# FangjinhuaWang/PatchmatchNet

Hardware: AMD Instinct MI355X
Metric: depth-maps/sec at 1600x1200 N=5 src views (higher is better)
Workload: dtype f32

## Files before the change

include/pmn_hip.h:

```cpp
#ifndef PMN_HIP_H
#define PMN_HIP_H

#include <stdint.h>

#ifdef __cplusplus
extern "C" {
#endif

#define PMN_ABI_VERSION 25
#define PMN_MLP_FLOATS 340
#define PMN_MAX_DEPTH 64
#define PMN_MAX_NEIGHBORS 17
#define PMN_MAX_FUSE_SRC 32
#define PMN_TSDF_MAX_VIEWS 16
#define PMN_TSDF_MARK_SPAN 8
#define PMN_RASTER_MAX_DIM 16384
#define PMN_RASTER_MAX_BOX 64
#define PMN_SPLAT_MAX_RADIUS 32

#define PMN_OK 0
#define PMN_ERR_ARG (-1)
#define PMN_ERR_SHAPE (-2)
#define PMN_ERR_LAUNCH (-3)

int pmn_abi_version(void);

const char *pmn_error_string(int code);

int pmn_nchw_to_nhwc(const float *in, float *out, int B, int C, int h, int w, void *stream);

int pmn_feature_weight(const float *ref_nhwc, const float *eval_offsets, const int *eval_table_host,
                       const float *mlp, int B, int C, int G, int K, int h, int w,
                       float *out_feature_weight, void *stream);

int pmn_init_hypotheses(const float *noise, const float *depth, int depth_shift, const float *depth_min,
                        const float *depth_max, int num_sample, float interval_scale, const float *propa_offsets,
                        const int *propa_table_host, int K, int B, int h, int w, float *depth_sample,
                        float *xnorm, void *stream);

int pmn_warp_correlate(const float *ref_nhwc, const float *src_nhwc, const float *rel_proj,
                       const float *depth_sample, const float *view_weights_in, int vw_shift,
                       const float *similarity_mlp, const float *pixelwise_mlp, int B, int N, int C,
                       int G, int D, int h, int w, int hs, int ws, float *cost_out, float *view_weights_out,
                       int *vw_argmax_out, float *similarity_out, void *stream);

int pmn_warp_correlate_views(const float *ref_nhwc, const void *src_view_table, const float *rel_proj,
                             const float *depth_sample, const float *view_weights_in, int vw_shift,
                             const float *similarity_mlp, const float *pixelwise_mlp, int B, int N, int C,
                             int G, int D, int h, int w, int hs, int ws, float *cost_out, float *view_weights_out,
                             int *vw_argmax_out, float *similarity_out, void *stream);

int pmn_aggregate_regress(const float *cost, const float *depth_sample, const float *xnorm,
                          const float *feature_weight, const float *eval_offsets, const int *eval_table_host,
                          int K, float interval_scale, int is_inverse, int B, int D, int h, int w,
                          float *score_out, float *depth_out, void *stream);

int pmn_confidence(const float *score, int B, int D, int h, int w, int H, int W, float *confidence_out,
                   int *depth_index_out, void *stream);

int pmn_conv2d(const float *in, const float *weights, const float *shift, const float *up, float *out, int N, int H,
               int W, int cin, int cout, int K, int stride, int pad, int dil, int relu, int in_nchw, int out_nchw,
               int up_h, int up_w, void *stream);

int pmn_fpn_tail(const float *x, const float *up, const float *w_in, const float *b_in, const float *w_out, float *out,
                 int N, int H, int W, int cin, int cmid, int cout, void *stream);

int pmn_conv2d_mfma(const float *in, const float *weights, const float *shift, float *out, float *out_b, int N, int H, int W,
                    int cin, int cout, int ca, int K, int stride, int pad, int dil, int relu, int planar, void *stream);


int pmn_conv2d_f16s(const float *in, const void *weights, const float *shift, float *out, int N, int H, int W, int cin, int cout,
                    int k, int stride, int relu, void *stream);

int pmn_conv2d_f16s_pair(const float *in, const void *weights_a, const float *shift_a, const void *weights_b, const float *shift_b,
                         float *out, int N, int H, int W, int channels, int relu, void *stream);

int pmn_offset_heads_f16s(const float *in, const void *weights, const float *shift, float *out_a, float *out_b, int N, int H, int W,
                          int cin, int cout, int ca, int dil, void *stream);

int pmn_fpn_level(const float *x, const float *u, const float *w, const float *b, float *out_a, float *out_b, int N, int H,
                  int W, int cin, int cout, int ca, void *stream);

int pmn_deconv3x3s2(const float *in, const float *weights, const float *shift, float *out, int N, int Hi, int Wi, int cin,
                    int cout, int relu, void *stream);

int pmn_refine_front(const float *img, const float *t2, const float *w0, const float *s0, const float *wd, const float *sd,
                     float *x16, int B, int H, int W, void *stream);
int pmn_refine_tail(const float *x16, const float *w3, const float *s3, const float *wr, const float *dnorm,
                    const float *depth_min, const float *depth_max, float *out, int B, int H, int W, void *stream);

int pmn_refine_fused(const float *img, const float *t2, const float *w0, const float *s0, const float *wd, const float *sd,
                     const void *w3a, const float *s3, const float *wr, const float *dnorm, const float *depth_min,
                     const float *depth_max, float *out, int B, int H, int W, void *stream);

int pmn_stage_projections(const float *intrinsics, const float *extrinsics, int B, int V, int nstages, float scale0,
                          float *rel, void *stream);

int pmn_stem(const float *img, const float *w0, const float *s0, const float *w1, const float *s1, float *out, int N, int H,
             int W, void *stream);

int pmn_stem_f16s(const float *img, const float *w0, const float *s0, const void *w1a, const float *s1, float *out, int N, int H,
                  int W, void *stream);

int pmn_stem_f16s_views(const float *const *img_table, int views, const float *w0, const float *s0, const void *w1a,
                        const float *s1, float *out, int B, int H, int W, void *stream);

int pmn_stem_conv2_f16s(const float *img, const float *w0, const float *s0, const void *w1a, const float *s1, const void *w2b,
                        const float *s2, float *out, int N, int H, int W, void *stream);

int pmn_stem_conv2_f16s_views(const float *const *img_table, int views, const float *w0, const float *s0, const void *w1a,
                              const float *s1, const void *w2b, const float *s2, float *out, int B, int H, int W, void *stream);

int pmn_differentiable_warping(const float *src_nchw, const float *rel_proj, const float *depth, int B, int C,
                               int D, int h, int w, int hs, int ws, float *warped, void *stream);

int pmn_fuse_view(const float *maps, long long slot_stride, int ref_slot, const int *src_slots_host,
                  const int *src_hw_host, int n_src, const float *mats, int H, int W, float geo_pixel_thres, float geo_depth_thres, int geo_mask_thres,
                  float photo_thres, unsigned char *masks, float *xyz, double *depth_avg, int *geo_sum, void *stream);

int pmn_fuse_view_merged(const float *maps, long long slot_stride, int ref_slot, const int *src_slots_host,
                         const int *src_hw_host, int n_src, const float *mats, int H, int W, float geo_pixel_thres,
// ... 197 lines not shown
```

patchmatchnet_amd/_lib.py:

```python
from __future__ import annotations

import ctypes
import os
import subprocess
from typing import Optional

_CSRC = os.path.join(os.path.dirname(os.path.abspath(__file__)), "csrc")
LIB_PATH = os.path.join(_CSRC, "libpmn_hip.so")
ABI_VERSION = 25
MLP_FLOATS = 340
MAX_DEPTH = 64
MAX_NEIGHBORS = 17
MAX_FUSE_SRC = 32
TSDF_MAX_VIEWS = 16
TSDF_MARK_SPAN = 8
RASTER_MAX_DIM = 16384
RASTER_MAX_BOX = 64
SPLAT_MAX_RADIUS = 32
ICP_SUMS = 17
ICP_LIMBS = 5
ICP_BLOCK_POINTS = 256
VOXEL_LONG_RUN = 256
VOXEL_MAX_CHANNELS = 8
CROP_MAX_VERTICES = 4096
MESH_PLACE_LONG_RUN = 256
MESH_SIMPLIFY_MAX_FACES = 715827882
MESH_SMOOTH_LONG_ROW = 256
MESH_SMOOTH_MAX_STEPS = 65536
NORMAL_SWEEPS = 6
NORMAL_MAX_VIEWPOINTS = 4096
PLANE_MAX_HYPOTHESES = 4096
PLANE_SUMS = 10
PLANE_LIMBS = 5
PLANE_BLOCK_POINTS = 1024
MLS_QUADRIC_MIN = 6
MLS_PIVOT_MIN = 1e-10

_fp = ctypes.c_void_p
_ip = ctypes.c_void_p
_hp = ctypes.c_void_p
_i = ctypes.c_int
_f = ctypes.c_float
_s = ctypes.c_void_p

SIGNATURES = {
    "pmn_abi_version": [],
    "pmn_error_string": [_i],
    "pmn_nchw_to_nhwc": [_fp, _fp, _i, _i, _i, _i, _s],
    "pmn_feature_weight": [_fp, _fp, _hp, _fp, _i, _i, _i, _i, _i, _i, _fp, _s],
    "pmn_init_hypotheses": [_fp, _fp, _i, _fp, _fp, _i, _f, _fp, _hp, _i, _i, _i, _i, _fp, _fp, _s],
    "pmn_warp_correlate": [_fp, _fp, _fp, _fp, _fp, _i, _fp, _fp, _i, _i, _i, _i, _i, _i, _i, _i, _i, _fp, _fp, _ip,
                           _fp, _s],
    "pmn_warp_correlate_views": [_fp, _fp, _fp, _fp, _fp, _i, _fp, _fp, _i, _i, _i, _i, _i, _i, _i, _i, _i, _fp, _fp, _ip,
                                 _fp, _s],
    "pmn_aggregate_regress": [_fp, _fp, _fp, _fp, _fp, _hp, _i, _f, _i, _i, _i, _i, _i, _fp, _fp, _s],
    "pmn_confidence": [_fp, _i, _i, _i, _i, _i, _i, _fp, _ip, _s],
    "pmn_conv2d": [_fp, _fp, _fp, _fp, _fp] + [_i] * 14 + [_s],
    "pmn_fpn_tail": [_fp] * 6 + [_i] * 6 + [_s],
    "pmn_fpn_level": [_fp] * 6 + [_i] * 6 + [_s],
    "pmn_conv2d_f16s": [_fp] * 4 + [_i] * 8 + [_s],
    "pmn_offset_heads_f16s": [_fp] * 5 + [_i] * 7 + [_s],
    "pmn_conv2d_f16s_pair": [_fp] * 6 + [_i] * 5 + [_s],
    "pmn_refine_front": [_fp] * 7 + [_i] * 3 + [_s],
    "pmn_refine_tail": [_fp] * 8 + [_i] * 3 + [_s],
    "pmn_refine_fused": [_fp] * 13 + [_i] * 3 + [_s],
    "pmn_conv2d_mfma": [_fp] * 5 + [_i] * 12 + [_s],
    "pmn_deconv3x3s2": [_fp] * 4 + [_i] * 6 + [_s],
    "pmn_stage_projections": [_fp, _fp, _i, _i, _i, _f, _fp, _s],
    "pmn_stem": [_fp] * 6 + [_i] * 3 + [_s],
    "pmn_stem_f16s": [_fp] * 6 + [_i] * 3 + [_s],
    "pmn_stem_f16s_views": [_fp, _i] + [_fp] * 5 + [_i] * 3 + [_s],
    "pmn_stem_conv2_f16s": [_fp] * 8 + [_i] * 3 + [_s],
    "pmn_stem_conv2_f16s_views": [_fp, _i] + [_fp] * 7 + [_i] * 3 + [_s],
    "pmn_differentiable_warping": [_fp, _fp, _fp, _i, _i, _i, _i, _i, _i, _i, _fp, _s],
    "pmn_fuse_view": [_fp, ctypes.c_longlong, _i, _hp, _hp, _i, _fp, _i, _i, _f, _f, _i, _f, _fp, _fp, _fp, _ip, _s],
    "pmn_fuse_view_merged": [_fp, ctypes.c_longlong, _i, _hp, _hp, _i, _fp, _i, _i, _f, _f, _i, _f, _fp, _fp, _fp, _ip, _fp,
                             ctypes.c_longlong, _fp, _s],
    "pmn_pack_points": [_fp, _fp, _fp, _i, _i, _i, _fp, ctypes.c_longlong, _fp, _ip, _fp, _s],
    "pmn_pack_points_normals": [_fp, _fp, _fp, _fp, _i, _fp, _i, _i, _i, _fp, ctypes.c_longlong, _fp, _ip, _fp, _s],
    "pmn_depth_normals": [_fp, _i, _i, _hp, _i, _f, _fp, _s],
    "pmn_normalize_depth": [_fp, _fp, _fp, _i, _i, _fp, _s],
    "pmn_check_f16_domain": [_fp, ctypes.c_longlong, _ip, _s],
    "pmn_plan_create": [ctypes.POINTER(ctypes.c_void_p)],
    "pmn_plan_begin": [_hp],
    "pmn_plan_end": [_hp],
    "pmn_plan_count": [_hp],
    "pmn_plan_kernel_name": [_hp, _i],
    "pmn_plan_launch": [_hp, _s],
    "pmn_plan_destroy": [_hp],
    "pmn_plan_fork": [_hp],
    "pmn_plan_switch": [_hp, _i],
    "pmn_plan_join": [_hp],
    "pmn_plan_entry_branch": [_hp, _i],
    "pmn_plan_launch_part": [_hp, _i, _s],
    "pmn_view_scores": [_fp] * 6 + [_i, _i, ctypes.c_longlong, ctypes.c_longlong] + [ctypes.c_double] * 3 + [_fp, _s],
    "pmn_depth_metrics": [_fp, _fp, _hp, _hp, _hp, _i, _hp, _i, _i, _i, _i, _fp, ctypes.c_longlong, _fp, _s],
    "pmn_nn_distance": [_fp, _ip, ctypes.c_longlong, _hp, ctypes.c_double, _hp, _fp, _ip, ctypes.c_longlong, ctypes.c_double, _fp, _ip,
                        _s],
    "pmn_reduce_round": [_fp, _ip, ctypes.c_longlong, _hp, ctypes.c_double, _hp, ctypes.c_double, _ip, _ip, _ip, _s],
    "pmn_tsdf_integrate": [_fp] * 4 + [_hp, _hp, _f, _f, _fp, ctypes.c_longlong] + [_hp] * 5 + [_i, _s],
    "pmn_mt_count": [_fp, _fp, _hp, _f, _ip, _ip, _s],
    "pmn_mt_emit": [_fp] * 4 + [_hp, _hp, _f, _f] + [_ip] * 4 + [_fp, _ip, _fp, _ip, _s],
    "pmn_tsdf_mark_blocks": [_ip, _ip, _hp, _hp, _f, _f, _fp, ctypes.c_longlong] + [_hp] * 4 + [_i, _s],
    "pmn_tsdf_integrate_blocks": [_fp] * 4 + [_ip, _i, _hp, _hp, _f, _f, _fp, ctypes.c_longlong] + [_hp] * 5 + [_i, _s],
    "pmn_mt_count_blocks": [_fp, _fp, _ip, _ip, _i, _hp, _f, _ip, _ip, _s],
    "pmn_mt_emit_blocks": [_fp] * 4 + [_ip, _ip, _i, _hp, _hp, _f, _f] + [_ip] * 4 + [_fp, _ip, _fp, _ip, _s],
    "pmn_raster_triangles": [_fp, _i, _ip, _i, _hp, _i, _i, ctypes.c_longlong, _ip, _ip, _ip, _s],
    "pmn_splat_points": [_fp, ctypes.c_longlong, _hp, _i, _i, _f, _f, _ip, _ip, _s],
    "pmn_raster_resolve": [_ip, _i, _i, _hp, _fp, ctypes.c_longlong, _ip, ctypes.c_longlong, _ip, _fp, _i, _fp, _ip, _ip, _fp, _s],
    "pmn_icp_accumulate": [_fp, _ip, ctypes.c_longlong, _hp, ctypes.c_double, _hp, _fp, _ip, ctypes.c_longlong, _hp, _hp, ctypes.c_double,
                           _fp, ctypes.c_longlong, _fp, _s],
    "pmn_voxel_mean": [_fp, _fp, _i, ctypes.c_longlong, _ip, ctypes.c_longlong, _fp, _fp, _s],
    "pmn_crop_prism": [_fp, ctypes.c_longlong, _fp, _i, _i, ctypes.c_double, ctypes.c_double, _hp, _ip, _s],
    "pmn_mesh_components": [_ip, _i, _i, _ip, _ip, _s],
    "pmn_mesh_face_samples": [_fp, _i, _ip, _i, ctypes.c_double, ctypes.c_ulonglong, _ip, _ip, _s],
    "pmn_mesh_sample": [_fp, _i, _ip, _i, _ip, _ip, ctypes.c_longlong, ctypes.c_ulonglong, _fp, _ip, _ip, _s],
    "pmn_undistort_image": [_fp, _i, _i, _i, _i, _hp, _hp, _i, _i, _fp, _fp, _fp, _s],
    "pmn_knn_distance": [_fp, _ip, ctypes.c_longlong, _hp, ctypes.c_double, _hp, _fp, _ip, ctypes.c_longlong, _i, ctypes.c_double, _i,
                         _fp, _ip, _fp, _s],
    "pmn_radius_count": [_fp, _ip, ctypes.c_longlong, _hp, ctypes.c_double, _hp, _fp, _ip, ctypes.c_longlong, ctypes.c_double, _i, _ip,
                         _s],
    "pmn_knn_normals": [_fp, _ip, ctypes.c_longlong, _hp, ctypes.c_double, _hp, _fp, _ip, ctypes.c_longlong, _i, ctypes.c_double, _i,
                        _fp, _i, ctypes.c_double, _fp, _fp, _ip, _s],
    "pmn_cloud_core": [_fp, _ip, ctypes.c_longlong, _hp, ctypes.c_double, _hp, ctypes.c_double, ctypes.c_longlong, _ip, _s],
    "pmn_cloud_dbscan": [_fp, _ip, ctypes.c_longlong, _hp, ctypes.c_double, _hp, ctypes.c_double, _ip, _ip, _ip, _ip, _s],
    "pmn_plane_score": [_fp, _fp, _ip, ctypes.c_longlong, _fp, _i, ctypes.c_double, ctypes.c_double, _ip, _s],
    "pmn_plane_inliers": [_fp, _fp, _ip, ctypes.c_longlong, _hp, ctypes.c_double, ctypes.c_double, _hp, _hp, _fp, ctypes.c_longlong, _ip,
                          _fp, _s],
    "pmn_cloud_sdf_blocks": [_fp, _ip, ctypes.c_longlong, _hp, ctypes.c_double, _hp, _fp, _ip, _ip, _i, _hp, _hp, _f, _f, _i,
                             ctypes.c_double, ctypes.c_double, _fp, _fp, _fp, _fp, _s],
    "pmn_knn_mls": [_fp, _ip, ctypes.c_longlong, _hp, ctypes.c_double, _hp, _fp, _ip, ctypes.c_longlong, _i, ctypes.c_double, _i, _i,
                    ctypes.c_double, _fp, _fp, _fp, _ip, _ip, _s],
    "pmn_mesh_distance": [_fp, _ip, ctypes.c_longlong, _hp, ctypes.c_double, _hp, _ip, ctypes.c_double, _fp, _i, _ip, _i, _fp, _ip,
# ... 80 lines not shown
```

patchmatchnet_amd/csrc/hypotheses.hip:

```cpp
#include <cstring>

#include "pmn_common.hpp"
#define PMN_DIV48(u) ((u) / 48.0f)
#define PMN_DIV48R(u) pmn_div_by((u), 48.0f, r48)

struct HypArgs {
    const float* noise;
    const float* depth;
    const float* depth_min;
    const float* depth_max;
    const float* offsets;
    float* depth_sample;
    float* xnorm;
    int depth_shift, num_sample, K, B, h, w;
    float interval_scale;
    int table[2 * PMN_MAX_NEIGHBORS];
};

__device__ __forceinline__ float centre_hypothesis(const HypArgs& a, int b, int qy, int qx, float inv_min, float inv_max,
                                                   float interval, int kc) {
#pragma clang fp contract(off)
    const int h = a.h, w = a.w;
    if (a.noise) {
        const float u = a.noise[((size_t)b * 48 + 24) * h * w + (size_t)qy * w + qx] + 24.0f;
// ... 155 lines not shown
                v[j] = pmn_div(1.0f, inv);
            }
        }
    }

    if constexpr (KT > 0) {
        constexpr int KB = KT < 8 ? KT : 8;
        static_assert(KT % KB == 0, "whole batches");
        const float* cbase = from_noise ? a.noise + ((size_t)b * 48 + 24) * hw
                                        : a.depth + (size_t)b * (h >> a.depth_shift) * ws;
        const int sh = from_noise ? 0 : a.depth_shift, cw = from_noise ? w : ws;
#pragma unroll
        for (int k0b = 0; k0b < KT; k0b += KB) {
            float ox[KB], oy[KB];
#pragma unroll
            for (int i = 0; i < KB; ++i) {
                ox[i] = a.offsets[((size_t)b * 2 * KT + 2 * (k0b + i)) * hw + p];
                oy[i] = a.offsets[((size_t)b * 2 * KT + 2 * (k0b + i) + 1) * hw + p];
            }
            PmnTaps t[KB];
            float c[KB][4];
#pragma unroll
            for (int i = 0; i < KB; ++i) {
                float ix, iy;
                pmn_neighbor_position((float)x, (float)y, a.table[2 * (k0b + i)], a.table[2 * (k0b + i) + 1], ox[i], oy[i], h, w, ix,
                                      iy);
                t[i] = pmn_make_taps(ix, iy, h, w);
                const int qy = t[i].off / w, qx = t[i].off - qy * w;
                c[i][0] = cbase[(size_t)(qy >> sh) * cw + (qx >> sh)];
                c[i][1] = cbase[(size_t)(qy >> sh) * cw + ((qx + 1) >> sh)];
                c[i][2] = cbase[(size_t)((qy + 1) >> sh) * cw + (qx >> sh)];
                c[i][3] = cbase[(size_t)((qy + 1) >> sh) * cw + ((qx + 1) >> sh)];
            }
#pragma unroll
            for (int i = 0; i < KB; ++i) {
                float cc[4];
#pragma unroll
                for (int q = 0; q < 4; ++q) {
                    if (from_noise) {
                        const float inv = inv_max + PMN_DIV48R(c[i][q] + 24.0f) * (inv_min - inv_max);
                        cc[q] = pmn_div(1.0f, inv);
                    } else if (a.num_sample == 1) {
                        cc[q] = c[i][q];
                    } else {
                        float inv = pmn_div(1.0f, c[i][q]) + interval * (float)kc;
                        inv = fminf(fmaxf(inv, inv_max), inv_min);
                        cc[q] = pmn_div(1.0f, inv);
                    }
                }
                v[D0T + k0b + i] = fmaf(cc[3], t[i].w11, fmaf(cc[2], t[i].w10, fmaf(cc[1], t[i].w01, cc[0] * t[i].w00)));
            }
        }
#pragma unroll
        for (int kk = 2; kk <= NP2; kk <<= 1) {
#pragma unroll
            for (int jj = kk >> 1; jj > 0; jj >>= 1) {
#pragma unroll
                for (int i = 0; i < NP2; ++i) {
                    const int l = i ^ jj;
                    if (l > i) {
                        const float lo = fminf(v[i], v[l]), hi = fmaxf(v[i], v[l]);
                        if ((i & kk) == 0) {
                            v[i] = lo;
                            v[l] = hi;
                        } else {
                            v[i] = hi;
                            v[l] = lo;
                        }
                    }
                }
            }
        }
    }

    const float range = inv_min - inv_max, rrange = pmn_rcp_refined(range);
#pragma unroll
    for (int j = 0; j < D; ++j) {
        const size_t o = ((size_t)b * D + j) * hw + p;
        a.depth_sample[o] = v[j];
        a.xnorm[((size_t)b * hw + p) * D + j] = pmn_div_by(pmn_div(1.0f, v[j]) - inv_max, range, rrange);
    }
}

extern "C" int pmn_init_hypotheses(const float* noise, const float* depth, int depth_shift, const float* depth_min,
                                   const float* depth_max, int num_sample, float interval_scale,
                                   const float* propa_offsets, const int* propa_table_host, int K, int B, int h, int w,
                                   float* depth_sample, float* xnorm, void* stream) {
    if ((!noise && !depth) || !depth_min || !depth_max || !depth_sample || !xnorm) return PMN_ERR_ARG;
    if (B < 1 || h < 2 || w < 2 || K < 0 || depth_shift < 0 || depth_shift > 1) return PMN_ERR_ARG;
    if (K > 0 && (!propa_offsets || !propa_table_host)) return PMN_ERR_ARG;
    if (K > 16) return PMN_ERR_SHAPE;
    if (!noise && num_sample < 1) return PMN_ERR_ARG;
    if (depth_shift && ((h | w) & 1)) return PMN_ERR_ARG;
    const int D0 = noise ? 48 : num_sample;
    const int D = D0 + K;
    if (D > PMN_MAX_DEPTH) return PMN_ERR_SHAPE;
    HypArgs a;
    memset(&a, 0, sizeof(a));
    a.noise = noise;
    a.depth = noise ? nullptr : depth;
    a.depth_min = depth_min;
    a.depth_max = depth_max;
    a.offsets = propa_offsets;
    a.depth_sample = depth_sample;
    a.xnorm = xnorm;
    a.depth_shift = depth_shift;
    a.num_sample = noise ? 48 : num_sample;
    a.K = K;
    a.B = B; a.h = h; a.w = w;
    a.interval_scale = interval_scale;
    for (int i = 0; i < 2 * K; ++i) a.table[i] = propa_table_host[i];
    const int bs = (h * w <= 64 * 1024) ? 64 : PMN_BLOCK;
    const dim3 grid((h * w + bs - 1) / bs, B), block(bs);
    hipStream_t s = (hipStream_t)stream;
    if (noise && K == 16) PMN_LAUNCH((init_hypotheses_fixed_kernel<64, 48, 16>), grid, block, 0, s, a);
    else if (!noise && num_sample == 16 && K == 16) PMN_LAUNCH((init_hypotheses_fixed_kernel<32, 16, 16>), grid, block, 0, s, a);
    else if (!noise && num_sample == 8 && K == 8) PMN_LAUNCH((init_hypotheses_fixed_kernel<16, 8, 8>), grid, block, 0, s, a);
    else if (!noise && num_sample == 8 && K == 0) PMN_LAUNCH((init_hypotheses_fixed_kernel<8, 8, 0>), grid, block, 0, s, a);
    else if (D <= 8) PMN_LAUNCH(init_hypotheses_kernel<8>, grid, block, 0, s, a);
    else if (D <= 16) PMN_LAUNCH(init_hypotheses_kernel<16>, grid, block, 0, s, a);
    else if (D <= 32) PMN_LAUNCH(init_hypotheses_kernel<32>, grid, block, 0, s, a);
    else PMN_LAUNCH(init_hypotheses_kernel<64>, grid, block, 0, s, a);
    PMN_CHECK_LAUNCH();
    return PMN_OK;
}
```

patchmatchnet_amd/ops.py:

```python
from __future__ import annotations

import ctypes
import threading
from typing import List, Optional, Sequence, Tuple

import numpy as np
import torch

from . import _lib
from ._lib import PmnError, check


_TIMING = None
_TIMING_ON = True


def enable_kernel_timing() -> None:
    global _TIMING, _TIMING_ON
    _TIMING, _TIMING_ON = [], True


def pause_kernel_timing(paused: bool) -> None:
    global _TIMING_ON
    _TIMING_ON = not paused
# ... 197 lines not shown
        if v.is_contiguous():
            return v
        x = x.contiguous()
    _dev(x, "x")
    B, C, h, w = x.shape
    if out is None:
        out = torch.empty((B, h, w, C), dtype=torch.float32, device=x.device)
    else:
        _dev(out, "out")
        if tuple(out.shape) != (B, h, w, C):
            raise PmnError("nchw_to_nhwc: bad output shape")
    _note((x,), (out,))
    with torch.cuda.device(x.device):
        check(_lib.lib().pmn_nchw_to_nhwc(x.data_ptr(), out.data_ptr(), B, C, h, w, _stream(x)), "pmn_nchw_to_nhwc")
    return out


def stack_sources_nhwc(src_features: Sequence[torch.Tensor]) -> torch.Tensor:
    buf, sizes = stack_sources_padded(src_features)
    if any(sz != sizes[0] for sz in sizes):
        raise PmnError("all source feature maps of one stage must share a shape (stack_sources_padded handles mixed sizes)")
    return buf


def stack_sources_padded(src_features: Sequence[torch.Tensor]):
    if len(src_features) == 0:
        raise PmnError("at least one source view is required")
    B, C = src_features[0].shape[:2]
    sizes = [(int(f.shape[2]), int(f.shape[3])) for f in src_features]
    if any(tuple(f.shape[:2]) != (B, C) for f in src_features):
        raise PmnError("source feature maps of one stage must share batch size and channels")
    hs, ws = max(h for h, _ in sizes), max(w for _, w in sizes)
    mixed = any(sz != (hs, ws) for sz in sizes)
    alloc = torch.zeros if mixed else torch.empty
    buf = alloc((len(src_features), B, hs, ws, C), dtype=torch.float32, device=src_features[0].device)
    for i, f in enumerate(src_features):
        v = f.permute(0, 2, 3, 1)
        if sizes[i] != (hs, ws):
            _dev(f.contiguous(), "src_feature")
            buf[i][:, :sizes[i][0], :sizes[i][1], :].copy_(v)
        elif f.is_cuda and f.dtype == torch.float32 and v.is_contiguous():
            buf[i].copy_(v)
        else:
            nchw_to_nhwc(f.contiguous(), buf[i])
    return buf, sizes


def rescale_projection_rows(rel_proj: torch.Tensor, sizes, padded_hw) -> torch.Tensor:
    HS, WS = padded_hw
    if all(sz == (HS, WS) for sz in sizes):
        return rel_proj
    out = rel_proj.clone()
    for v, (h_v, w_v) in enumerate(sizes):
        if (h_v, w_v) != (HS, WS):
            out[:, v, 0, :] *= (w_v - 1) / (WS - 1)
            out[:, v, 1, :] *= (h_v - 1) / (HS - 1)
    return out.contiguous()


def _mlp_dev(t: torch.Tensor, name: str) -> torch.Tensor:
    _dev(t, name)
    if t.numel() != _lib.MLP_FLOATS:
        raise PmnError(f"{name}: expected a packed MLP block of {_lib.MLP_FLOATS} floats")
    return t


def feature_weight(ref_nhwc: torch.Tensor, eval_offsets: torch.Tensor, table: np.ndarray, mlp: torch.Tensor,
                   G: int) -> torch.Tensor:
    _dev(ref_nhwc, "ref_nhwc")
    _dev(eval_offsets, "eval_offsets")
    B, h, w, C = ref_nhwc.shape
    K = eval_offsets.shape[1] // 2
    if tuple(eval_offsets.shape) != (B, 2 * K, h, w):
        raise PmnError("feature_weight: eval_offsets must be [B,2K,h,w]")
    tab, tab_p = _host_i32(table, 2 * K, "table")
    _mlp_dev(mlp, "mlp")
    out = torch.empty((B, K, h, w), dtype=torch.float32, device=ref_nhwc.device)
    _note((ref_nhwc, eval_offsets, mlp), (out,))
    with torch.cuda.device(ref_nhwc.device):
        check(_lib.lib().pmn_feature_weight(ref_nhwc.data_ptr(), eval_offsets.data_ptr(), tab_p, mlp.data_ptr(), B, C, G,
                                            K, h, w,
                                            out.data_ptr(), _stream(out)), "pmn_feature_weight")
    return out


def init_hypotheses(noise: Optional[torch.Tensor], depth: Optional[torch.Tensor], depth_shift: int,
                    depth_min: torch.Tensor, depth_max: torch.Tensor, num_sample: int, interval_scale: float,
                    propa_offsets: Optional[torch.Tensor], table: Optional[np.ndarray], h: int, w: int
                    ) -> Tuple[torch.Tensor, torch.Tensor]:
    _dev(depth_min, "depth_min")
    _dev(depth_max, "depth_max")
    B = depth_min.shape[0]
    dev = depth_min.device
    if noise is not None:
        _dev(noise, "noise")
        if tuple(noise.shape) != (B, 48, h, w):
            raise PmnError("init_hypotheses: noise must be [B,48,h,w]")
        D0 = 48
    else:
        if depth is None:
            raise PmnError("init_hypotheses: need noise or depth")
        _dev(depth, "depth")
        if tuple(depth.shape) != (B, 1, h >> depth_shift, w >> depth_shift):
            raise PmnError(f"init_hypotheses: depth must be [B,1,{h >> depth_shift},{w >> depth_shift}], "
                           f"got {tuple(depth.shape)}")
        D0 = num_sample
    K = 0
    tab_p = None
    tab = None
    if propa_offsets is not None:
        _dev(propa_offsets, "propa_offsets")
        K = propa_offsets.shape[1] // 2
        if tuple(propa_offsets.shape) != (B, 2 * K, h, w):
            raise PmnError("init_hypotheses: propa_offsets must be [B,2K,h,w]")
        tab, tab_p = _host_i32(table, 2 * K, "table")
    D = D0 + K
    ds = torch.empty((B, D, h, w), dtype=torch.float32, device=dev)
    xn = torch.empty((B, h, w, D), dtype=torch.float32, device=dev).permute(0, 3, 1, 2)
    _note((noise, depth if noise is None else None, depth_min, depth_max, propa_offsets), (ds, xn))
    with torch.cuda.device(dev):
        check(_lib.lib().pmn_init_hypotheses(_ptr(noise), _ptr(depth) if noise is None else None, depth_shift,
                                             depth_min.data_ptr(), depth_max.data_ptr(), num_sample,
                                             float(interval_scale), _ptr(propa_offsets), tab_p, K, B, h, w,
                                             ds.data_ptr(), xn.data_ptr(), _stream(ds)), "pmn_init_hypotheses")
    del tab
    return ds, xn


class SourceTable:

    def __init__(self, table: torch.Tensor, shape) -> None:
        if table.dtype != torch.int64 or not table.is_cuda or table.numel() != int(shape[0]):
            raise PmnError("SourceTable: int64 device tensor with one address per source view")
        self.table, self.shape, self.device = table, tuple(int(x) for x in shape), table.device

    @staticmethod
    def image_in_place(im: torch.Tensor) -> bool:
        return bool(im.is_cuda and im.dtype == torch.float32 and im.is_contiguous() and im.data_ptr() % 16 == 0)

    @staticmethod
    def addresses(maps) -> list:
        out = []
        for m in maps:
            if not (m.is_cuda and m.dtype == torch.float32 and m.is_contiguous()):
                raise PmnError("SourceTable: dense float32 channels-last device maps")
            out.append(m.data_ptr())
        return out


def warp_correlate(ref_nhwc: torch.Tensor, src_nhwc, rel_proj: torch.Tensor, depth_sample: torch.Tensor,
                   view_weights: Optional[torch.Tensor], vw_shift: int, similarity_mlp: torch.Tensor,
                   pixelwise_mlp: Optional[torch.Tensor], G: int, want_similarity: bool = False,
                   want_argmax: bool = False):
    _dev(ref_nhwc, "ref_nhwc")
    table = src_nhwc if isinstance(src_nhwc, SourceTable) else None
    if table is None:
        _dev(src_nhwc, "src_nhwc")
    _dev(rel_proj, "rel_proj")
    _dev(depth_sample, "depth_sample")
    B, h, w, C = ref_nhwc.shape
    N, Bs, hs, ws, Cs = src_nhwc.shape
    D = depth_sample.shape[1]
    if Bs != B or Cs != C or tuple(depth_sample.shape) != (B, D, h, w) or tuple(rel_proj.shape) != (B, N, 4, 4):
        raise PmnError("warp_correlate: inconsistent shapes")
    dev = ref_nhwc.device
    sim_p = _mlp_dev(similarity_mlp, "similarity_mlp").data_ptr()
    pix_p, vw_out, argmax = None, None, None
    if view_weights is not None:
        _dev(view_weights, "view_weights")
        if tuple(view_weights.shape) != (B, N, h >> vw_shift, w >> vw_shift):
            raise PmnError("Patchmatch Evaluation: Different number of images and view weights")
    else:
        if pixelwise_mlp is None:
            raise PmnError("warp_correlate: pixelwise_mlp required when view_weights is None")
        pix_p = _mlp_dev(pixelwise_mlp, "pixelwise_mlp").data_ptr()
        vw_out = torch.empty((B, N, h, w), dtype=torch.float32, device=dev)
        if want_argmax:
            argmax = torch.empty((B, N, h, w), dtype=torch.int32, device=dev)
    cost = torch.empty((B, h, w, D), dtype=torch.float32, device=dev).permute(0, 3, 1, 2)
    sim = torch.empty((B, G, D, h, w), dtype=torch.float32, device=dev) if want_similarity else None
    _note((ref_nhwc, src_nhwc if table is None else table.table, rel_proj, depth_sample, view_weights, similarity_mlp, pixelwise_mlp),
          (cost, vw_out, argmax, sim))
    with torch.cuda.device(dev):
        if _TIMING is not None and _TIMING_ON:
            ev0, ev1 = torch.cuda.Event(enable_timing=True), torch.cuda.Event(enable_timing=True)
            ev0.record()
        fn = _lib.lib().pmn_warp_correlate if table is None else _lib.lib().pmn_warp_correlate_views
        check(fn(ref_nhwc.data_ptr(), (src_nhwc if table is None else table.table).data_ptr(), rel_proj.data_ptr(),
                 depth_sample.data_ptr(), _ptr(view_weights), vw_shift, sim_p, pix_p, B, N, C,
                 G, D, h, w, hs, ws, cost.data_ptr(), _ptr(vw_out), _ptr(argmax), _ptr(sim),
                 _stream(cost)), "pmn_warp_correlate")
        if _TIMING is not None and _TIMING_ON:
            ev1.record()
            _TIMING.append((ev0, ev1, 4 * B * h * w * ((1 + N) * C + D + N + G * D),
                            f"C{C}_D{D}_{h}x{w}_N{N}_{'vw' if view_weights is not None else 'pixelwise'}"))
    return cost, (view_weights if view_weights is not None else vw_out), argmax, sim


def aggregate_regress(cost: torch.Tensor, depth_sample: torch.Tensor, xnorm: torch.Tensor, feature_weight_: torch.Tensor,
                      eval_offsets: torch.Tensor, table: np.ndarray, interval_scale: float, is_inverse: bool
                      ) -> Tuple[torch.Tensor, torch.Tensor]:
    for n, t in (("depth_sample", depth_sample), ("feature_weight", feature_weight_), ("eval_offsets", eval_offsets)):
        _dev(t, n)
    cost, xnorm = _dlast(cost, "cost"), _dlast(xnorm, "xnorm")
    B, D, h, w = cost.shape
    K = feature_weight_.shape[1]
    if tuple(depth_sample.shape) != (B, D, h, w) or tuple(xnorm.shape) != (B, D, h, w) or \
# ... 1136 lines not shown
```

Before: 408.4.

## Split hypothesis init across lanes with DPP bitonic sort and vectorised xnorm stores

Adds a hypothesis-initialisation kernel that spreads each pixel's depth hypotheses across 1, 2 or 4 lanes of a quad. The bitonic sort uses DPP lane swaps and fmed3 selects, and the xnorm rows are written with float4 stores. The Python wrapper now calls the new path-selecting entry point with the default path, so the supported shape combinations use the lane-split kernel. The aim is to cut per-thread register pressure and serial sorting work in the large 64-hypothesis case and to coalesce stores. The cost is extra complexity and more threads per pixel.

Measured after the change: 410.1, median of 6. About the same (+0.4%).

```diff
diff --git a/include/pmn_hip.h b/include/pmn_hip.h
--- a/include/pmn_hip.h
+++ b/include/pmn_hip.h
@@ -37,6 +37,16 @@
                         const float *depth_max, int num_sample, float interval_scale, const float *propa_offsets,
                         const int *propa_table_host, int K, int B, int h, int w, float *depth_sample,
                         float *xnorm, void *stream);
+
+#define PMN_HYP_PATH_THREAD 0
+#define PMN_HYP_PATH_DEFAULT 1
+#define PMN_HYP_PATH_EXPLICIT 0x100
+#define PMN_HYP_PATH_VEC4 0x10
+#define PMN_HYP_PATH_ONE_WAVE 0x20
+int pmn_init_hypotheses_path(const float *noise, const float *depth, int depth_shift, const float *depth_min,
+                             const float *depth_max, int num_sample, float interval_scale, const float *propa_offsets,
+                             const int *propa_table_host, int K, int B, int h, int w, float *depth_sample,
+                             float *xnorm, int path, void *stream);
 
 int pmn_warp_correlate(const float *ref_nhwc, const float *src_nhwc, const float *rel_proj,
                        const float *depth_sample, const float *view_weights_in, int vw_shift,
diff --git a/patchmatchnet_amd/_lib.py b/patchmatchnet_amd/_lib.py
--- a/patchmatchnet_amd/_lib.py
+++ b/patchmatchnet_amd/_lib.py
@@ -35,6 +35,11 @@
 PLANE_BLOCK_POINTS = 1024
 MLS_QUADRIC_MIN = 6
 MLS_PIVOT_MIN = 1e-10
+HYP_PATH_THREAD = 0
+HYP_PATH_DEFAULT = 1
+HYP_PATH_EXPLICIT = 0x100
+HYP_PATH_VEC4 = 0x10
+HYP_PATH_ONE_WAVE = 0x20
 
 _fp = ctypes.c_void_p
 _ip = ctypes.c_void_p
@@ -49,6 +54,7 @@
     "pmn_nchw_to_nhwc": [_fp, _fp, _i, _i, _i, _i, _s],
     "pmn_feature_weight": [_fp, _fp, _hp, _fp, _i, _i, _i, _i, _i, _i, _fp, _s],
     "pmn_init_hypotheses": [_fp, _fp, _i, _fp, _fp, _i, _f, _fp, _hp, _i, _i, _i, _i, _fp, _fp, _s],
+    "pmn_init_hypotheses_path": [_fp, _fp, _i, _fp, _fp, _i, _f, _fp, _hp, _i, _i, _i, _i, _fp, _fp, _i, _s],
     "pmn_warp_correlate": [_fp, _fp, _fp, _fp, _fp, _i, _fp, _fp, _i, _i, _i, _i, _i, _i, _i, _i, _i, _fp, _fp, _ip,
                            _fp, _s],
     "pmn_warp_correlate_views": [_fp, _fp, _fp, _fp, _fp, _i, _fp, _fp, _i, _i, _i, _i, _i, _i, _i, _i, _i, _fp, _fp, _ip,
diff --git a/patchmatchnet_amd/csrc/hypotheses.hip b/patchmatchnet_amd/csrc/hypotheses.hip
--- a/patchmatchnet_amd/csrc/hypotheses.hip
+++ b/patchmatchnet_amd/csrc/hypotheses.hip
@@ -261,10 +261,208 @@
     }
 }
 
+template <int M>
+__device__ __forceinline__ float hyp_lane_xor(float v) {
+    static_assert(M == 1 || M == 2, "a permutation within a quad");
+    return __int_as_float(__builtin_amdgcn_mov_dpp(__float_as_int(v), M == 1 ? 0xB1 : 0x4E, 0xF, 0xF, true));
+}
+
+__device__ __forceinline__ float hyp_pick(float x, float y, float s) { return __builtin_amdgcn_fmed3f(x, y, s); }
+
+template <int NP2, int LPI>
+__device__ __forceinline__ void hyp_sort_lanes(float (&v)[NP2 / LPI], int l) {
+    constexpr int R = NP2 / LPI, LANE_LO = 4, LANE_HI = 4 * LPI;
+    const float inf = __builtin_inff();
+#pragma unroll
+    for (int kk = 2; kk <= NP2; kk <<= 1) {
+        const bool kk_lane = kk >= LANE_LO && kk < LANE_HI;
+        const bool desc_lane = kk_lane && (l & (kk >> 2)) != 0;
+#pragma unroll
+        for (int jj = kk >> 1; jj > 0; jj >>= 1) {
+            if (jj >= LANE_LO && jj < LANE_HI) {
+                const bool upper = (l & (jj >> 2)) != 0;
+#pragma unroll
+                for (int r = 0; r < R; ++r) {
+                    const bool desc = kk_lane ? desc_lane : ((((r >> 2) * LANE_HI) & kk) != 0);
+                    const float o = jj == 4 ? hyp_lane_xor<1>(v[r]) : hyp_lane_xor<2>(v[r]);
+                    v[r] = hyp_pick(v[r], o, upper != desc ? inf : -inf);
+                }
+            } else {
+                const int rj = jj < LANE_LO ? jj : jj / LPI;
+#pragma unroll
+                for (int r = 0; r < R; ++r) {
+                    if ((r & rj) != 0) continue;
+                    const int r2 = r | rj;
+                    if (kk_lane) {
+                        const float x = v[r], y = v[r2];
+                        v[r] = hyp_pick(x, y, desc_lane ? inf : -inf);
+                        v[r2] = hyp_pick(x, y, desc_lane ? -inf : inf);
+                    } else {
+                        const float lo = fminf(v[r], v[r2]), hi = fmaxf(v[r], v[r2]);
+                        const bool desc = ((((r & 3) | ((r >> 2) * LANE_HI)) & kk) != 0);
+                        v[r] = desc ? hi : lo;
+                        v[r2] = desc ? lo : hi;
+                    }
+                }
+            }
+        }
+    }
+}
+
+template <int NP2, int D0T, int KT, int LPI, bool VEC4>
+__global__ __launch_bounds__(PMN_BLOCK) void init_hypotheses_lanes_kernel(const HypArgs a) {
+#pragma clang fp contract(off)
+    static_assert(LPI == 1 || LPI == 2 || LPI == 4, "a lane group is a part of a quad");
+    static_assert(D0T + KT == NP2, "no padding: every position is a hypothesis");
+    static_assert(D0T % LPI == 0 && KT % LPI == 0 && (NP2 / LPI) % 4 == 0, "whole runs of four per lane");
+    constexpr int D = NP2, R = NP2 / LPI, RL = D0T / LPI, RK = KT / LPI, LB = LPI == 4 ? 2 : LPI == 2 ? 1 : 0;
+    const int h = a.h, w = a.w, hw = h * w;
+    const int t = blockIdx.x * blockDim.x + threadIdx.x;
+    const int p = t / LPI, l = t % LPI;
+    const int b = blockIdx.y;
+    if (p >= hw) return;
+    const int y = p / w, x = p - y * w;
+    const float inv_min = 1.0f / a.depth_min[b];
+    const float inv_max = 1.0f / a.depth_max[b];
+    const float interval = (inv_min - inv_max) * a.interval_scale;
+    const int k0 = -((a.num_sample + 1) / 2);
+    const int kc = k0 + a.num_sample / 2;
+    const bool from_noise = a.noise != nullptr;
+    const float r48 = pmn_uniform(pmn_rcp_refined(48.0f));
+
+    float v[R];
+    const int ws = w >> a.depth_shift;
+    if (from_noise) {
+        float u[RL];
+#pragma unroll
+        for (int i = 0; i < RL; ++i) u[i] = a.noise[((size_t)b * 48 + (i * LPI + l)) * hw + p];
+#pragma unroll
+        for (int i = 0; i < RL; ++i) {
+            const float inv = inv_max + PMN_DIV48R(u[i] + (float)(i * LPI + l)) * (inv_min - inv_max);
+            v[i] = pmn_div(1.0f, inv);
+        }
+    } else {
+        const float dprev =
+            a.depth[(size_t)b * (h >> a.depth_shift) * ws + (size_t)(y >> a.depth_shift) * ws + (x >> a.depth_shift)];
+        const float inv_prev = pmn_div(1.0f, dprev);
+#pragma unroll
+        for (int i = 0; i < RL; ++i) {
+            float inv = inv_prev + interval * (float)(k0 + (i * LPI + l));
+            inv = fminf(fmaxf(inv, inv_max), inv_min);
+            v[i] = pmn_div(1.0f, inv);
+        }
+    }
+
+    if constexpr (KT > 0) {
+        constexpr int KB = RK < 8 ? RK : 8;
+        static_assert(RK % KB == 0, "whole batches");
+        const float* cbase = from_noise ? a.noise + ((size_t)b * 48 + 24) * hw
+                                        : a.depth + (size_t)b * (h >> a.depth_shift) * ws;
+        const int sh = from_noise ? 0 : a.depth_shift, cw = from_noise ? w : ws;
+#pragma unroll
+        for (int i0 = 0; i0 < RK; i0 += KB) {
+            float ox[KB], oy[KB];
+#pragma unroll
+            for (int i = 0; i < KB; ++i) {
+                const int k = (i0 + i) * LPI + l;
+                ox[i] = a.offsets[((size_t)b * 2 * KT + 2 * k) * hw + p];
+                oy[i] = a.offsets[((size_t)b * 2 * KT + 2 * k + 1) * hw + p];
+            }
+            PmnTaps t4[KB];
+            float c[KB][4];
+#pragma unroll
+            for (int i = 0; i < KB; ++i) {
+                int dy = a.table[2 * (i0 + i) * LPI], dx = a.table[2 * (i0 + i) * LPI + 1];
+#pragma unroll
+                for (int q = 1; q < LPI; ++q)
+                    if (l == q) {
+                        dy = a.table[2 * ((i0 + i) * LPI + q)];
+                        dx = a.table[2 * ((i0 + i) * LPI + q) + 1];
+                    }
+                float ix, iy;
+                pmn_neighbor_position((float)x, (float)y, dy, dx, ox[i], oy[i], h, w, ix, iy);
+                t4[i] = pmn_make_taps(ix, iy, h, w);
+                const int qy = t4[i].off / w, qx = t4[i].off - qy * w;
+                c[i][0] = cbase[(size_t)(qy >> sh) * cw + (qx >> sh)];
+                c[i][1] = cbase[(size_t)(qy >> sh) * cw + ((qx + 1) >> sh)];
+                c[i][2] = cbase[(size_t)((qy + 1) >> sh) * cw + (qx >> sh)];
+                c[i][3] = cbase[(size_t)((qy + 1) >> sh) * cw + ((qx + 1) >> sh)];
+            }
+#pragma unroll
+            for (int i = 0; i < KB; ++i) {
+                float cc[4];
+#pragma unroll
+                for (int q = 0; q < 4; ++q) {
+                    if (from_noise) {
+                        const float inv = inv_max + PMN_DIV48R(c[i][q] + 24.0f) * (inv_min - inv_max);
+                        cc[q] = pmn_div(1.0f, inv);
+                    } else {
+                        float inv = pmn_div(1.0f, c[i][q]) + interval * (float)kc;
+                        inv = fminf(fmaxf(inv, inv_max), inv_min);
+                        cc[q] = pmn_div(1.0f, inv);
+                    }
+                }
+                v[RL + i0 + i] = fmaf(cc[3], t4[i].w11, fmaf(cc[2], t4[i].w10, fmaf(cc[1], t4[i].w01, cc[0] * t4[i].w00)));
+            }
+        }
+        hyp_sort_lanes<NP2, LPI>(v, l);
+    }
+
+    const float range = inv_min - inv_max, rrange = pmn_rcp_refined(range);
+    float* xrow = a.xnorm + ((size_t)b * hw + p) * D;
+#pragma unroll
+    for (int q = 0; q < R / 4; ++q) {
+        const int s0 = (l << 2) | (q << (2 + LB));
+        float xn[4];
+#pragma unroll
+        for (int e = 0; e < 4; ++e) {
+            a.depth_sample[((size_t)b * D + s0 + e) * hw + p] = v[4 * q + e];
+            xn[e] = pmn_div_by(pmn_div(1.0f, v[4 * q + e]) - inv_max, range, rrange);
+        }
+        if (VEC4) {
+            *reinterpret_cast<float4*>(xrow + s0) = make_float4(xn[0], xn[1], xn[2], xn[3]);
+        } else {
+#pragma unroll
+            for (int e = 0; e < 4; ++e) xrow[s0 + e] = xn[e];
+        }
+    }
+}
+
+template <int NP2, int D0T, int KT>
+static int hyp_launch_lanes(const HypArgs& a, int lpi, bool vec4, bool one_wave, hipStream_t s) {
+    const size_t threads = (size_t)a.h * a.w * lpi;
+    const int bs = (one_wave || threads <= 64 * 1024) ? 64 : PMN_BLOCK;
+    const dim3 grid((unsigned)((threads + bs - 1) / bs), a.B), block(bs);
+#define PMN_HYP_LANES(L)                                                                                              \
+    if (lpi == L) {                                                                                                   \
+        if (vec4) PMN_LAUNCH((init_hypotheses_lanes_kernel<NP2, D0T, KT, L, true>), grid, block, 0, s, a);            \
+        else PMN_LAUNCH((init_hypotheses_lanes_kernel<NP2, D0T, KT, L, false>), grid, block, 0, s, a);                \
+        PMN_CHECK_LAUNCH();                                                                                           \
+        return PMN_OK;                                                                                                \
+    }
+    PMN_HYP_LANES(1)
+    if constexpr (NP2 >= 16) {
+        PMN_HYP_LANES(2)
+        PMN_HYP_LANES(4)
+    }
+#undef PMN_HYP_LANES
+    return PMN_ERR_ARG;
+}
+
 extern "C" int pmn_init_hypotheses(const float* noise, const float* depth, int depth_shift, const float* depth_min,
                                    const float* depth_max, int num_sample, float interval_scale,
                                    const float* propa_offsets, const int* propa_table_host, int K, int B, int h, int w,
                                    float* depth_sample, float* xnorm, void* stream) {
+    return pmn_init_hypotheses_path(noise, depth, depth_shift, depth_min, depth_max, num_sample, interval_scale, propa_offsets,
+                                    propa_table_host, K, B, h, w, depth_sample, xnorm, PMN_HYP_PATH_THREAD, stream);
+}
+
+extern "C" int pmn_init_hypotheses_path(const float* noise, const float* depth, int depth_shift, const float* depth_min,
+                                        const float* depth_max, int num_sample, float interval_scale,
+                                        const float* propa_offsets, const int* propa_table_host, int K, int B, int h, int w,
+                                        float* depth_sample, float* xnorm, int path, void* stream) {
+    if (path != PMN_HYP_PATH_THREAD && path != PMN_HYP_PATH_DEFAULT && !(path & PMN_HYP_PATH_EXPLICIT)) return PMN_ERR_ARG;
+    if ((path & PMN_HYP_PATH_EXPLICIT) && (path & ~(PMN_HYP_PATH_EXPLICIT | 7 | PMN_HYP_PATH_VEC4 | PMN_HYP_PATH_ONE_WAVE))) return PMN_ERR_ARG;
     if ((!noise && !depth) || !depth_min || !depth_max || !depth_sample || !xnorm) return PMN_ERR_ARG;
     if (B < 1 || h < 2 || w < 2 || K < 0 || depth_shift < 0 || depth_shift > 1) return PMN_ERR_ARG;
     if (K > 0 && (!propa_offsets || !propa_table_host)) return PMN_ERR_ARG;
@@ -289,9 +487,24 @@
     a.B = B; a.h = h; a.w = w;
     a.interval_scale = interval_scale;
     for (int i = 0; i < 2 * K; ++i) a.table[i] = propa_table_host[i];
+    hipStream_t s = (hipStream_t)stream;
+    const int combo = (noise && K == 16) ? 0 : (!noise && num_sample == 16 && K == 16) ? 1 : (!noise && num_sample == 8 && K == 8) ? 2
+                    : (!noise && num_sample == 8 && K == 0) ? 3 : -1;
+    if (combo >= 0 && path != PMN_HYP_PATH_THREAD) {
+        static const int default_lanes[4] = {4, 4, 2, 1};
+        const bool expl = (path & PMN_HYP_PATH_EXPLICIT) != 0;
+        const int lpi = expl ? (path & 7) : default_lanes[combo];
+        const bool vec4 = (expl ? (path & PMN_HYP_PATH_VEC4) != 0 : true) && ((uintptr_t)xnorm & 15) == 0;
+        const bool one_wave = expl && (path & PMN_HYP_PATH_ONE_WAVE);
+        switch (combo) {
+            case 0: return hyp_launch_lanes<64, 48, 16>(a, lpi, vec4, one_wave, s);
+            case 1: return hyp_launch_lanes<32, 16, 16>(a, lpi, vec4, one_wave, s);
+            case 2: return hyp_launch_lanes<16, 8, 8>(a, lpi, vec4, one_wave, s);
+            default: return hyp_launch_lanes<8, 8, 0>(a, lpi, vec4, one_wave, s);
+        }
+    }
     const int bs = (h * w <= 64 * 1024) ? 64 : PMN_BLOCK;
     const dim3 grid((h * w + bs - 1) / bs, B), block(bs);
-    hipStream_t s = (hipStream_t)stream;
     if (noise && K == 16) PMN_LAUNCH((init_hypotheses_fixed_kernel<64, 48, 16>), grid, block, 0, s, a);
     else if (!noise && num_sample == 16 && K == 16) PMN_LAUNCH((init_hypotheses_fixed_kernel<32, 16, 16>), grid, block, 0, s, a);
     else if (!noise && num_sample == 8 && K == 8) PMN_LAUNCH((init_hypotheses_fixed_kernel<16, 8, 8>), grid, block, 0, s, a);
diff --git a/patchmatchnet_amd/ops.py b/patchmatchnet_amd/ops.py
--- a/patchmatchnet_amd/ops.py
+++ b/patchmatchnet_amd/ops.py
@@ -303,6 +303,9 @@
                                             K, h, w,
                                             out.data_ptr(), _stream(out)), "pmn_feature_weight")
     return out
+
+
+hypotheses_path = _lib.HYP_PATH_DEFAULT
 
 
 def init_hypotheses(noise: Optional[torch.Tensor], depth: Optional[torch.Tensor], depth_shift: int,
@@ -340,10 +343,11 @@
     xn = torch.empty((B, h, w, D), dtype=torch.float32, device=dev).permute(0, 3, 1, 2)
     _note((noise, depth if noise is None else None, depth_min, depth_max, propa_offsets), (ds, xn))
     with torch.cuda.device(dev):
-        check(_lib.lib().pmn_init_hypotheses(_ptr(noise), _ptr(depth) if noise is None else None, depth_shift,
-                                             depth_min.data_ptr(), depth_max.data_ptr(), num_sample,
-                                             float(interval_scale), _ptr(propa_offsets), tab_p, K, B, h, w,
-                                             ds.data_ptr(), xn.data_ptr(), _stream(ds)), "pmn_init_hypotheses")
+        check(_lib.lib().pmn_init_hypotheses_path(_ptr(noise), _ptr(depth) if noise is None else None, depth_shift,
+                                                  depth_min.data_ptr(), depth_max.data_ptr(), num_sample,
+                                                  float(interval_scale), _ptr(propa_offsets), tab_p, K, B, h, w,
+                                                  ds.data_ptr(), xn.data_ptr(), int(hypotheses_path), _stream(ds)),
+              "pmn_init_hypotheses_path")
     del tab
     return ds, xn
 
```
